# Hunger-Prevails/3D-Pose-Estimation-with-Previleged-Information

Hardware: AMD Instinct MI355X
Metric: crops/sec (fwd+bwd) ResNet-50 pose head, 256x256 bs=64/GPU (higher is better)
Workload: dtype f32 (3xbf16 split, 6 products, f32 accumulate); 1 GPU; depthnet resnet50 pose head, 256x256 crops, batch 64/GPU, full step: fwd + soft-argmax + SmoothL1 + bwd + RCCL grad all-reduce + clip + Adam; global_batch=64, parallelism=dp1, dist_world_size=1, wgrad_stream_runs_beside_launch_stream=True

## Files before the change

### 3d-pose-estimation-with-previleged-information_amd/csrc/p3d_fx.hip

```cpp
#include <type_traits>
#include <mutex>
#include "p3d_common.h"
#include "p3d_fx.h"

namespace p3d {

using bf8 = __bf16 __attribute__((ext_vector_type(8)));
using f32x16 = float __attribute__((ext_vector_type(16)));
using f32x4 = float __attribute__((ext_vector_type(4)));
using f32x2 = float __attribute__((ext_vector_type(2)));
using u32x2 = unsigned __attribute__((ext_vector_type(2)));
using s4t = short __attribute__((ext_vector_type(4)));
using s8v = short __attribute__((ext_vector_type(8)));
using i32x4 = int __attribute__((ext_vector_type(4)));

constexpr int FX_BM = 128, FX_BN = 128, FX_BK = 16;
constexpr int FX_PIECE = 128 * FX_BK * 2;

using bf16x2 = __bf16 __attribute__((ext_vector_type(2)));
__device__ __forceinline__ unsigned fx_pack2(float a, float b) {
    const bf16x2 h = __builtin_convertvector(f32x2{a, b}, bf16x2);
    return __builtin_bit_cast(unsigned, h);
}
__device__ __forceinline__ void fx_split2(float x0, float x1, unsigned& hp, unsigned& mp, unsigned& lp) {
// ... 401 lines not shown
                    if (!split) {
                        const f32x4 c2 = *reinterpret_cast<const f32x4*>(p.ep_c + ((size_t)n * p.M + m) * OHW + rem);
#pragma unroll
                        for (int e = 0; e < 4; ++e) {
                            const float gg = fmaf(c2[e], esc[b], esh[b]) > 0.f ? v[e] : 0.f;
                            ssum[b] += gg; ssq[b] = fmaf(gg, c2[e] - emean[b], ssq[b]);
                        }
                    }
                }
            }
        }
    if (dense) {
        constexpr int EROW = 512 + 16;
        const bool accum = EPI != 3 && !split && p.accumulate;
#pragma unroll
        for (int b = 0; b < 2; ++b) {
            if (b == 1) __syncthreads();
#pragma unroll
            for (int a = 0; a < 2; ++a)
#pragma unroll
                for (int g = 0; g < 4; ++g)
                    *reinterpret_cast<f32x4*>(lds + (wm * 32 + fr) * EROW + (wn * 64 + a * 32 + 8 * g + 4 * fh) * 4) =
                        f32x4{acc[a][b][4 * g], acc[a][b][4 * g + 1], acc[a][b][4 * g + 2], acc[a][b][4 * g + 3]};
            __syncthreads();
#pragma unroll
            for (int i = 0; i < 8; ++i) {
                const int id = t + 256 * i, row = id >> 5, q = id & 31;
                const int m = m0 + (row >> 5) * 64 + b * 32 + (row & 31);
                const int c4 = n0 + 4 * q;
                if (m >= p.M || c4 >= p.NP) continue;
                const int n = c4 / OHW, rem = c4 - n * OHW;
                f32x4 v = *reinterpret_cast<const f32x4*>(lds + row * EROW + q * 16);
                const size_t at = ((size_t)n * p.M + m) * OHW + rem;
                f32x4* dst = reinterpret_cast<f32x4*>(yout + at);
                if (accum) {
                    f32x4 o4;
                    if (p.acc_src) {
                        o4 = *reinterpret_cast<const f32x4*>(p.acc_src + at);
                        if (p.acc_mask) {
                            const unsigned mk = p.acc_mask[at >> 2];
#pragma unroll
                            for (int e = 0; e < 4; ++e) o4[e] = (mk >> e) & 1u ? o4[e] : 0.f;
                        }
                    } else o4 = *dst;
                    v[0] += o4[0]; v[1] += o4[1]; v[2] += o4[2]; v[3] += o4[3];
                }
                if constexpr (EPIX == 8) {
                    if (p.ep_res) { const f32x4 r4 = *reinterpret_cast<const f32x4*>(p.ep_res + at); v[0] += r4[0]; v[1] += r4[1]; v[2] += r4[2]; v[3] += r4[3]; }
                    if (p.ep_relu) { v[0] = fmaxf(v[0], 0.f); v[1] = fmaxf(v[1], 0.f); v[2] = fmaxf(v[2], 0.f); v[3] = fmaxf(v[3], 0.f); }
                }
                *dst = v;
            }
        }
    }
    if constexpr (EPI == 1 || EPI == 2) {
        if (!split) {
#pragma unroll
            for (int b = 0; b < 2; ++b) {
                ssum[b] += __shfl_xor(ssum[b], 32, 64);
                ssq[b] += __shfl_xor(ssq[b], 32, 64);
                if (fh == 0) { red[wn][0][wm * 64 + b * 32 + fr] = ssum[b]; red[wn][1][wm * 64 + b * 32 + fr] = ssq[b]; }
            }
            __syncthreads();
            if (t < 128 && m0 + t < p.M) {
                float* dst = p.partial + ((size_t)tile_n * p.M + m0 + t) * 2;
                dst[0] = red[0][0][t] + red[1][0][t];
                dst[1] = red[0][1][t] + red[1][1][t];
            }
        }
    }
    if constexpr (EPI == 3) {
        float (*const red3)[3][128] = reinterpret_cast<float (*)[3][128]>(lds + 40960);
#pragma unroll
        for (int b = 0; b < 2; ++b) {
            ssum[b] += __shfl_xor(ssum[b], 32, 64);
            ssq[b] += __shfl_xor(ssq[b], 32, 64);
            sthird[b] += __shfl_xor(sthird[b], 32, 64);
            if (fh == 0) { const int ch = wm * 64 + b * 32 + fr; red3[wn][0][ch] = ssum[b]; red3[wn][1][ch] = ssq[b]; red3[wn][2][ch] = sthird[b]; }
        }
        __syncthreads();
        if (t < 128 && m0 + t < p.M)
            *reinterpret_cast<f32x4*>(p.tail_partial + ((size_t)tile_n * p.M + m0 + t) * 4) =
                f32x4{red3[0][0][t] + red3[1][0][t], red3[0][1][t] + red3[1][1][t], red3[0][2][t] + red3[1][2][t], 0.f};
    }
}

template <int BM, int EPI, bool TAPI = false>
__global__ __launch_bounds__(256, 3) void fx16_conv_kernel(const FxConvParams p_in) {
    const FxConvParams p = fx_class_params(p_in);
    static_assert(BM == 128 || BM == 96 || BM == 64, "channel tile");
    constexpr int GA = 4, GB = BM / 32;
    constexpr int WCH = BM / 2;
    constexpr int PIECE_P = 128 * 32, PIECE_C = BM * 32;
    constexpr int BUFB = 3 * PIECE_P + 3 * PIECE_C, CH0 = 3 * PIECE_P;
    constexpr int LDSB = 2 * BUFB > 43008 ? 2 * BUFB : 43008;
    __shared__ __attribute__((aligned(16))) unsigned char lds[LDSB];
    float (*const red)[2][128] = reinterpret_cast<float (*)[2][128]>(lds + 40960);
    const int t = threadIdx.x, lane = t & 63, wave = __builtin_amdgcn_readfirstlane(t >> 6), wm = wave >> 1, wn = wave & 1;
    int bid;
    {
        const int nwg = gridDim.x, q = nwg >> 3, r = nwg & 7, xcd = blockIdx.x & 7, idx = blockIdx.x >> 3;
        bid = (xcd < r ? xcd * (q + 1) : r * (q + 1) + (xcd - r) * q) + idx;
    }
    const int tiles_n_all = gridDim.x / p.tiles_m;
    const int tile_m = p.order ? bid / tiles_n_all : bid % p.tiles_m, tile_n = p.order ? bid % tiles_n_all : bid / p.tiles_m;
    const int m0 = tile_m * BM, n0 = tile_n * FX_BN;
    const int OHW = p.OH * p.OW;
    const int HWi = p.Hi * p.Wi;
    const int nfirst = n0 / OHW;
    const int csteps = p.Cred / FX_BK;
    const int tiles128 = (p.M + 127) >> 7;
    int nk = p.ntap * csteps, kt0 = 0;
    if (p.kchunk > 0) {
        kt0 = blockIdx.y * p.kchunk;
        nk = min(nk - kt0, p.kchunk);
    }
    int f_tap = kt0 / csteps, f_k = (kt0 - f_tap * csteps) * FX_BK;
    if constexpr (TAPI) { f_k = (kt0 / p.ntap) * FX_BK; f_tap = kt0 - (kt0 / p.ntap) * p.ntap; }

    const i32x4 rW = fx_rsrc(p.Wimg, (size_t)p.R * p.S * tiles128 * csteps * (3 * FX_PIECE));
    int w_voff[3], w_lds[3];
#pragma unroll
    for (int j = 0; j < 3; ++j) {
        const int id = t + 256 * j, pc = id / (2 * BM), i = id - pc * (2 * BM), row = i >> 1, half = i & 1;
        const int grow = m0 + row, tl = grow >> 7;
        const bool ok = pc < 3 && tl < tiles128;
        w_voff[j] = ok ? tl * csteps * (3 * FX_PIECE) + pc * FX_PIECE + fx_rc_off(grow & 127, half) : FX_OOB;
        w_lds[j] = CH0 + (pc < 3 ? pc : 0) * PIECE_C + 16 * i;
    }
    constexpr int WCHUNKS = (3 * 2 * BM + 255) / 256;
    const bool w_last = (3 * 2 * BM) % 256 == 0 || t + 256 * (WCHUNKS - 1) < 3 * 2 * BM;

    const int pp = t >> 1, ph = t & 1;
    const int col = n0 + pp;
    const bool col_ok = col < p.NP;
    int hbase = 0, wbase = 0, img_off = 0;
    {
        const int cc = col_ok ? col : 0;
        const int pn = cc / OHW;
        const int rem = cc - pn * OHW, oh = rem / p.OW, ow = rem - oh * p.OW;
        hbase = oh * p.hmul + p.hoff;
        wbase = ow * p.wmul + p.woff;
        img_off = (pn - nfirst) * csteps * HWi;
    }
    i32x4 rXi[3];
    {
        const size_t left = (size_t)(p.N - nfirst) * p.Cred * HWi * 2;
#pragma unroll
        for (int pc = 0; pc < 3; ++pc) rXi[pc] = fx_rsrc(p.Ximg + pc * p.plane_bytes + (size_t)nfirst * p.Cred * HWi * 2, left);
    }
    int x_voff = FX_OOB, w_tapoff = 0, cur_tap = -1;
    auto set_tap = [&](int tap) {
        cur_tap = tap;
        const int ir = tap / p.nS, is = tap - ir * p.nS;
        const int wtap = (p.r0 + p.rstep * ir) * p.S + p.s0 + p.sstep * is;
        w_tapoff = wtap * tiles128 * csteps * (3 * FX_PIECE);
        const int hi = hbase + ir * p.hstep, wi0 = wbase + is * p.wstep;
        const bool ok = col_ok && (unsigned)hi < (unsigned)p.Hi && (unsigned)wi0 < (unsigned)p.Wi;
        x_voff = ok ? (img_off + hi * p.Wi + wi0) * 32 + 16 * ph : FX_OOB;
    };
    i32x4 rwi[3], rxi[3];
    auto fetch = [&]() {
        if (f_tap != cur_tap) { asm volatile("" ::: "memory"); set_tap(f_tap); }
        {
            const int so = w_tapoff + (f_k >> 4) * (3 * FX_PIECE);
#pragma unroll
// ... 782 lines not shown
    }
    const FxPairSide a{c_a, (unsigned char*)img_a, fa->gamma, fa->dgamma, fa->dbeta, fa->table, pixmul_a}, b{c_b, (unsigned char*)img_b, fb->gamma, fb->dgamma, fb->dbeta, fb->table, nullptr};
    const dim3 grid((unsigned)ceil_div((int64_t)N * (HW >> 2) * 2, 256), (unsigned)(C >> 4));
    hipLaunchKernelGGL(fx_act_image_pair_kernel, grid, dim3(256), 0, st, x, gmask, a, b, (const double*)fa->partial, fa->rows, fa->count, fa->accumulate,
                       (size_t)N * C * HW * 2, N, C, HW);
    return check_launch("fx_act_image_pair");
}

size_t fx_act_image_bytes(int64_t N, int64_t C, int64_t HW) { return (size_t)(3 * N * C * HW * 2); }

int32_t fx_act_image(int mode, const float* x, const float* x2, const float* table, int masked, void* img, int N, int C, int HW, hipStream_t st,
                     const FxFinalize* fin, const float* pixmul) {
    if (!x || !img || N <= 0 || C <= 0 || (C & 15) || HW <= 0 || (HW & 3) || (mode != 0 && !table && !fin) || (mode == 2 && !x2) || mode < 0 || mode > 2) {
        set_error("fx_act_image: bad argument (N=%d C=%d HW=%d mode=%d; C %% 16 == 0 and HW %% 4 == 0 are required)", N, C, HW, mode); return P3D_EINVAL;
    }
    FxFinalize f{};
    if (fin) {
        f = *fin;
        if (!((f.kind == 1 && mode == 1 && f.beta) || ((f.kind == 2 || f.kind == 3) && mode == 2 && f.dgamma && f.dbeta)) || !f.partial || f.rows <= 0 || !f.gamma || !f.table) {
            set_error("fx_act_image: inconsistent fused-finalize request (kind %d, mode %d)", f.kind, mode); return P3D_EINVAL;
        }
    }
    const size_t plane = (size_t)N * C * HW * 2;
    const dim3 grid((unsigned)ceil_div((int64_t)N * (HW >> 2) * 2, 256), (unsigned)(C >> 4));
    if (mode == 0) hipLaunchKernelGGL(fx_act_image_kernel<0>, grid, dim3(256), 0, st, x, x2, table, (unsigned char*)img, plane, N, C, HW, masked, f, pixmul);
    else if (mode == 1) hipLaunchKernelGGL(fx_act_image_kernel<1>, grid, dim3(256), 0, st, x, x2, table, (unsigned char*)img, plane, N, C, HW, masked, f, pixmul);
    else hipLaunchKernelGGL(fx_act_image_kernel<2>, grid, dim3(256), 0, st, x, x2, table, (unsigned char*)img, plane, N, C, HW, masked, f, pixmul);
    return check_launch("fx_act_image");
}

static int g_fx = -1;
bool fx_enabled() {
    if (g_fx < 0) { const char* e = getenv("P3D_X3"); g_fx = (e && atoi(e) == 0) ? 0 : 1; }
    return g_fx == 1;
}
int fx_set_enabled(int on) { const int before = fx_enabled() ? 1 : 0; g_fx = on ? 1 : 0; return before; }

static std::mutex g_fx_count_mu;
static unsigned long long g_fx_count[6];
static double g_fx_flops[6];
void fx_count(int kind, const p3d_conv_desc* d) {
    std::lock_guard<std::mutex> lock(g_fx_count_mu);
    g_fx_count[kind] += 1;
    g_fx_flops[kind] += 2.0 * d->N * d->K * d->Ho * d->Wo * (double)d->C * d->R * d->S;
}
void fx_stats(unsigned long long* counts, double* flops, int reset) {
    std::lock_guard<std::mutex> lock(g_fx_count_mu);
    for (int i = 0; i < 6; ++i) { if (counts) counts[i] = g_fx_count[i]; if (flops) flops[i] = g_fx_flops[i]; }
    if (reset) for (int i = 0; i < 6; ++i) { g_fx_count[i] = 0; g_fx_flops[i] = 0.0; }
}

static bool fx_common(const p3d_conv_desc* d) {
    return fx_enabled() && d->c_offset >= 0 && d->c_offset + d->C <= d->c_total && d->R == d->S && (d->R & 1) && d->stride <= 2 &&
           (int64_t)d->N * d->C * d->H * d->W < (1ll << 31) && (int64_t)d->N * d->K * d->Ho * d->Wo < (1ll << 31) &&
           (int64_t)(d->K + 127) * (d->C + 127) * d->R * d->S * 6 < (1ll << 31);
}
bool fx_fwd_applies(const p3d_conv_desc* d, int min_m) {
    return fx_common(d) && d->C % FX_BK == 0 && d->C >= 32 && d->Wo % 4 == 0 && d->W % 4 == 0 && d->K >= min_m;
}
bool fx_dgrad_applies(const p3d_conv_desc* d, int min_m) {
    if (!(fx_common(d) && d->K % FX_BK == 0 && d->K >= 32 && d->C % 4 == 0 && d->C >= min_m && d->Wo % 4 == 0)) return false;
    if (d->stride == 1) return d->W % 4 == 0;
    return d->H % 2 == 0 && d->W % 8 == 0 && d->pad == d->dil * (d->R - 1) / 2 && (d->R == 1 || d->dil == 1);
}
bool fx_wgrad_applies(const p3d_conv_desc* d, int min_m) {
    if ((int64_t)d->N * d->C * d->H * d->W >= (1ll << 29) || (int64_t)d->N * d->K * d->Ho * d->Wo >= (1ll << 29)) return false;
    return fx_common(d) && d->K >= min_m && d->C >= min_m && (d->Ho * d->Wo) % FX_BK == 0 && d->Wo % 4 == 0 && d->W % 4 == 0 && (d->R == 1 || d->C % 64 == 0);
}

static int g_force_conv_splits = 0, g_force_wgrad_splits = 0, g_wgrad_target = 0;
static int g_tap_inner_min = [] { const char* e = getenv("P3D_TAP_INNER_MIN"); return e ? atoi(e) : 1024; }();
static int g_two_taps = 1;
static int g_conv_order = -1, g_wgrad_order = -1;
static int fx_conv_order(size_t wimg_bytes, int tiles_m, int tiles_n) {
    (void)wimg_bytes; (void)tiles_m; (void)tiles_n;
    return g_conv_order > 0 ? 1 : 0;
}
static int fx_wgrad_order(const p3d_conv_desc* d) {
    static const int env = [] { const char* e = getenv("P3D_WGRAD_ORDER"); return e ? atoi(e) : -1; }();
    const int forced = g_wgrad_order >= 0 ? g_wgrad_order : env;
    if (forced >= 0) return forced > 0 ? 1 : 0;
    return (d->R * d->S > 1 && d->C >= 512) ? 1 : 0;
}
static int g_class_launches = 0;
static int g_fx16 = -1;
static int fx16_mode() {
    if (g_fx16 < 0) { const char* e = getenv("P3D_FX16"); g_fx16 = e ? atoi(e) : 1; if (g_fx16 < 0 || g_fx16 > 2) g_fx16 = 1; }
    return g_fx16;
}
static int fx16_bm(int M, bool img, int pro, int epi) {
    const int mode = fx16_mode();
    if (epi == 5 || epi == 6 || epi == 7) epi = epi == 7 ? 0 : epi - 4;
    if (epi == 8) epi = 0;
    if (!img || pro != 0 || (epi != 0 && epi != 1 && epi != 2) || mode == 0) return 0;
    if (M <= 64) return 64;
    if (ceil_div(M, 96) * 96 < ceil_div(M, 128) * 128) return 96;
    return mode == 2 ? 128 : 0;
}
void fx_tune(int what, int value) {
    if (what == 3) { g_pair_map = value; return; }
    if (what == 5) { g_class_launches = value ? 1 : 0; return; }
    if (what == 9) { g_two_taps = value < 0 ? 1 : value; return; }
    if (what == 10) { g_tap_inner_min = value; return; }
    if (what == 7) { g_conv_order = value; return; }
    if (what == 8) { g_wgrad_order = value; return; }
    if (what == 4) { g_fx16 = value < 0 || value > 2 ? 1 : value; return; }
    (what == 0 ? g_force_wgrad_splits : what == 1 ? g_force_conv_splits : g_wgrad_target) = value;
}

struct FxSplit { int splits, kchunk; };
static FxSplit fx_plan_split(int64_t tiles, int nk) {
    FxSplit s{1, 0};
    int64_t want;
    if (g_force_conv_splits > 0) want = g_force_conv_splits < nk ? g_force_conv_splits : nk;
    else {
        static const int target = [] { const char* e = getenv("P3D_SPLITK_BLOCKS"); const int v = e ? atoi(e) : -1; return v >= 0 ? v : 768; }();
        if (tiles > 400 || nk < 64 || target == 0) return s;
        want = ceil_div(target, tiles);
        if (want > nk / 32) want = nk / 32;
        if (want > 8) want = 8;
    }
    if (want < 2) return s;
    s.kchunk = (int)ceil_div(nk, want);
    s.splits = (int)ceil_div(nk, s.kchunk);
    if (s.splits < 2) { s.splits = 1; s.kchunk = 0; }
    return s;
}

size_t fx_weight_image_bytes(int K, int C, int RS, bool bwd) {
    const int rows = bwd ? C : K, red = bwd ? K : C;
    return (size_t)RS * ((rows + 127) / 128) * (red / FX_BK) * (3 * FX_PIECE);
}
static size_t align256(size_t v) { return (v + 255) & ~(size_t)255; }

static FxSplit fx_fwd_split(const p3d_conv_desc* d) {
    return fx_plan_split(ceil_div(d->K, FX_BM) * ceil_div((int64_t)d->N * d->Ho * d->Wo, FX_BN), d->R * d->S * (d->C / FX_BK));
}
static FxSplit fx_dgrad_split(const p3d_conv_desc* d) {
    if (d->stride != 1) return FxSplit{1, 0};
    return fx_plan_split(ceil_div(d->C, FX_BM) * ceil_div((int64_t)d->N * d->H * d->W, FX_BN), d->R * d->S * (d->K / FX_BK));
}
static bool fx_masked_on() { static const bool on = [] { const char* e = getenv("P3D_FX_MASKED"); return !(e && atoi(e) == 0); }(); return on; }
bool fx_fwd_masked_applies(const p3d_conv_desc* d) { return fx_masked_on() && fx_fwd_applies(d, 64); }
bool fx_dgrad_masked_applies(const p3d_conv_desc* d) { return fx_masked_on() && fx_dgrad_applies(d, 64); }
bool fx_wgrad_masked_applies(const p3d_conv_desc* d) { return fx_masked_on() && fx_wgrad_applies(d, 96); }
size_t fx_fwd_workspace(const p3d_conv_desc* d) {
    const FxSplit s = fx_fwd_split(d);
    return align256(fx_weight_image_bytes(d->K, d->C, d->R * d->S, false)) + (s.splits > 1 ? (size_t)s.splits * d->N * d->K * d->Ho * d->Wo * sizeof(float) : 0);
}
size_t fx_dgrad_workspace(const p3d_conv_desc* d) {
    const FxSplit s = fx_dgrad_split(d);
    return align256(fx_weight_image_bytes(d->K, d->C, d->R * d->S, true)) + (s.splits > 1 ? (size_t)s.splits * d->N * d->C * d->H * d->W * sizeof(float) : 0);
}
int fx_partial_rows_fwd(const p3d_conv_desc* d) {
    const FxSplit s = fx_fwd_split(d);
    return s.splits > 1 ? (d->N < 16 ? d->N : 16) : (int)ceil_div((int64_t)d->N * d->Ho * d->Wo, FX_BN);
}
int fx_partial_rows_dgrad(const p3d_conv_desc* d) {
    const FxSplit s = fx_dgrad_split(d);
    return s.splits > 1 ? (d->N < 16 ? d->N : 16) : (int)ceil_div((int64_t)d->N * d->H * d->W, FX_BN);
}

__device__ __forceinline__ void fx_weight_image_chunks(const float* __restrict__ w, unsigned char* __restrict__ img, int K, int C, int RS, bool bwd, size_t first, size_t step,
                                                       int ctot, int coff, const float* __restrict__ scale = nullptr) {
    const int rows = bwd ? C : K, red = bwd ? K : C;
    const int tiles = (rows + 127) / 128, ksteps = red / FX_BK;
    const size_t total = (size_t)RS * tiles * ksteps * 256;
    for (size_t i = first; i < total; i += step) {
        const int half = (int)(i & 1), row = (int)((i >> 1) & 127);
        size_t j = i >> 8;
        const int ks = (int)(j % ksteps); j /= ksteps;
        const int tm = (int)(j % tiles);
        const int tap = (int)(j / tiles);
        const int m = tm * 128 + row, k0 = ks * FX_BK + half * 8;
        unsigned hi[8], mid[8], lo[8];
#pragma unroll
        for (int e = 0; e < 8; ++e) {
            float x = 0.f;
            if (m < rows) x = bwd ? w[((size_t)(k0 + e) * ctot + coff + m) * RS + tap] : w[((size_t)m * ctot + coff + k0 + e) * RS + tap];
            if (scale && m < rows) x = x * scale[m];
            const unsigned hb = __builtin_bit_cast(unsigned, x) & 0xFFFF0000u;
            const float r1 = x - __builtin_bit_cast(float, hb);
            const unsigned mb = __builtin_bit_cast(unsigned, r1) & 0xFFFF0000u;
            const float r2 = r1 - __builtin_bit_cast(float, mb);
            hi[e] = hb; mid[e] = mb; lo[e] = __builtin_bit_cast(unsigned, r2) & 0xFFFF0000u;
        }
        unsigned char* dst = img + (((size_t)tap * tiles + tm) * ksteps + ks) * (3 * FX_PIECE) + fx_rc_off(row, half);
        *reinterpret_cast<i32x4*>(dst) = i32x4{(int)((hi[0] >> 16) | hi[1]), (int)((hi[2] >> 16) | hi[3]), (int)((hi[4] >> 16) | hi[5]), (int)((hi[6] >> 16) | hi[7])};
        *reinterpret_cast<i32x4*>(dst + FX_PIECE) = i32x4{(int)((mid[0] >> 16) | mid[1]), (int)((mid[2] >> 16) | mid[3]), (int)((mid[4] >> 16) | mid[5]), (int)((mid[6] >> 16) | mid[7])};
        *reinterpret_cast<i32x4*>(dst + 2 * FX_PIECE) = i32x4{(int)((lo[0] >> 16) | lo[1]), (int)((lo[2] >> 16) | lo[3]), (int)((lo[4] >> 16) | lo[5]), (int)((lo[6] >> 16) | lo[7])};
    }
}
__global__ __launch_bounds__(256) void fx_weight_images_kernel(const float* __restrict__ w, unsigned char* __restrict__ img_fwd, unsigned char* __restrict__ img_bwd, int K,
                                                               int C, int RS, int ctot, int coff) {
    const bool bwd = blockIdx.y == 1;
    unsigned char* img = bwd ? img_bwd : img_fwd;
    if (img) fx_weight_image_chunks(w, img, K, C, RS, bwd, (size_t)blockIdx.x * 256 + threadIdx.x, (size_t)gridDim.x * 256, ctot, coff);
}
struct FxImageJob { const float* w; unsigned char* fwd; unsigned char* bwd; int K, C, RS, pad; };
__global__ __launch_bounds__(256) void fx_weight_images_batched_kernel(const FxImageJob* __restrict__ jobs) {
    const FxImageJob j = jobs[blockIdx.y >> 1];
    const bool bwd = blockIdx.y & 1;
    unsigned char* img = bwd ? j.bwd : j.fwd;
    if (img) fx_weight_image_chunks(j.w, img, j.K, j.C, j.RS, bwd, (size_t)blockIdx.x * 256 + threadIdx.x, (size_t)gridDim.x * 256, j.C, 0);
}
int32_t fx_build_weight_images_batched(const void* jobs, int njobs, int blocks, hipStream_t st) {
    static_assert(sizeof(FxImageJob) == 40, "job table layout (ops_block.py builds it)");
    if (njobs <= 0) return P3D_OK;
    hipLaunchKernelGGL(fx_weight_images_batched_kernel, dim3((unsigned)(blocks < 1 ? 1 : blocks), (unsigned)(2 * njobs)), dim3(256), 0, st, (const FxImageJob*)jobs);
    return check_launch("fx_build_weight_images_batched");
}

constexpr int FX_FOLD_MAX_K = 2048;
__global__ __launch_bounds__(256) void fx_fold_bn_kernel(const p3d_fold_job* __restrict__ jobs) {
    const p3d_fold_job j = jobs[blockIdx.y];
    __shared__ float sc[FX_FOLD_MAX_K];
    if (j.K <= 0 || j.K > FX_FOLD_MAX_K || j.C <= 0 || j.RS <= 0 || j.c_offset < 0 || j.c_offset + j.C > j.c_total || (j.kind == 0 && j.C % FX_BK != 0)) return;
    const bool bn = j.gamma != nullptr;
    for (int m = threadIdx.x; m < j.K; m += 256) {
        const float s = bn ? j.gamma[m] / sqrtf(j.var[m] + j.eps) : 1.f;
        sc[m] = s;
        if (blockIdx.x == 0 && j.bias_out) {
            float b = bn ? j.beta[m] - j.mean[m] * s : 0.f;
            if (j.conv_bias) b = bn ? b + s * j.conv_bias[m] : j.conv_bias[m];
            j.bias_out[m] = b;
        }
    }
    __syncthreads();
    const size_t first = (size_t)blockIdx.x * 256 + threadIdx.x, step = (size_t)gridDim.x * 256;
    if (j.kind == 0) {
        fx_weight_image_chunks(j.w, (unsigned char*)j.out, j.K, j.C, j.RS, false, first, step, j.c_total, j.c_offset, bn ? sc : nullptr);
    } else {
        float* out = (float*)j.out;
        const size_t per = (size_t)j.C * j.RS, total = (size_t)j.K * per;
        for (size_t i = first; i < total; i += step) {
            const int m = (int)(i / per);
            const size_t rest = i - (size_t)m * per;
            const int c = (int)(rest / j.RS), tap = (int)(rest - (size_t)c * j.RS);
            const float x = j.w[((size_t)m * j.c_total + j.c_offset + c) * j.RS + tap];
            out[i] = bn ? x * sc[m] : x;
        }
    }
}
int32_t fx_fold_bn_images(const void* jobs, int njobs, int blocks, hipStream_t st) {
    static_assert(sizeof(p3d_fold_job) == 96, "job table layout (infer.py builds it)");
    if (njobs <= 0) return P3D_OK;
    hipLaunchKernelGGL(fx_fold_bn_kernel, dim3((unsigned)(blocks < 1 ? 1 : blocks), (unsigned)njobs), dim3(256), 0, st, (const p3d_fold_job*)jobs);
    return check_launch("fx_fold_bn_images");
}

int32_t fx_build_weight_images(const float* w, int K, int C, int RS, void* img_fwd, void* img_bwd, hipStream_t st, int ctot, int coff) {
    if (ctot <= 0) { ctot = C; coff = 0; }
    const size_t a = img_fwd ? fx_weight_image_bytes(K, C, RS, false) / 48 : 0, b = img_bwd ? fx_weight_image_bytes(K, C, RS, true) / 48 : 0;
    const size_t total = a > b ? a : b;
    if (total == 0) return P3D_OK;
    const unsigned blocks = (unsigned)(ceil_div((int64_t)total, 256) < 4096 ? ceil_div((int64_t)total, 256) : 4096);
    hipLaunchKernelGGL(fx_weight_images_kernel, dim3(blocks, 2), dim3(256), 0, st, w, (unsigned char*)img_fwd, (unsigned char*)img_bwd, K, C, RS, ctot, coff);
    return check_launch("fx_build_weight_images");
}

static void fx_launch_conv(const FxConvParams& p_in, bool img, int pro, int epi, int bm, dim3 grid, hipStream_t st) {
    const int am = img ? 1 : 0;
    FxConvParams p = p_in;
    if (p.tap_inner && !((bm == 0 && am == 1 && pro == 0 && epi >= 0 && epi <= 2) || (bm == 96 && epi >= 0 && epi <= 2))) p.tap_inner = 0;
    if (p.tap_inner) {
#define P3D_FX_TAPI(EPI) if (bm == 0 && epi == EPI) { hipLaunchKernelGGL((fx_conv_kernel<1, 0, EPI, true>), grid, dim3(256), 0, st, p); return; } \
                         if (bm == 96 && epi == EPI) { hipLaunchKernelGGL((fx16_conv_kernel<96, EPI, true>), grid, dim3(256), 0, st, p); return; }
        P3D_FX_TAPI(0) P3D_FX_TAPI(1) P3D_FX_TAPI(2)
#undef P3D_FX_TAPI
    }
#define P3D_FX16_CASE(BM, EPI) if (bm == BM && (epi == EPI || epi == (EPI == 0 ? 7 : EPI + 4))) { hipLaunchKernelGGL((fx16_conv_kernel<BM, EPI>), grid, dim3(256), 0, st, p); return; }
    P3D_FX16_CASE(128, 0) P3D_FX16_CASE(128, 1) P3D_FX16_CASE(128, 2)
    P3D_FX16_CASE(96, 0) P3D_FX16_CASE(96, 1) P3D_FX16_CASE(96, 2)
    P3D_FX16_CASE(64, 0) P3D_FX16_CASE(64, 1) P3D_FX16_CASE(64, 2)
    P3D_FX16_CASE(128, 8) P3D_FX16_CASE(96, 8) P3D_FX16_CASE(64, 8)
#undef P3D_FX16_CASE
#define P3D_FX_CASE(AM, PRO, EPI) if (am == AM && pro == PRO && epi == EPI) { hipLaunchKernelGGL((fx_conv_kernel<AM, PRO, EPI>), grid, dim3(256), 0, st, p); return; }
    P3D_FX_CASE(0, 0, 0) P3D_FX_CASE(0, 0, 1) P3D_FX_CASE(0, 0, 2) P3D_FX_CASE(0, 4, 0) P3D_FX_CASE(0, 4, 4) P3D_FX_CASE(0, 4, 5)
    P3D_FX_CASE(1, 0, 0) P3D_FX_CASE(1, 0, 1) P3D_FX_CASE(1, 0, 2) P3D_FX_CASE(1, 0, 3) P3D_FX_CASE(1, 0, 5) P3D_FX_CASE(1, 0, 6) P3D_FX_CASE(1, 0, 7)
    P3D_FX_CASE(0, 0, 8) P3D_FX_CASE(1, 0, 8)
#undef P3D_FX_CASE
    set_error("fx_launch_conv: no kernel instance for img=%d pro=%d epi=%d bm=%d", am, pro, epi, bm);
}

static void fx_launch_reduce(int epi, dim3 grid, hipStream_t st, const float* slabs, float* y, const float* bias, int nsplit, size_t slab_stride, int N, int M,
                             int OHW, int accumulate, const float* ep_c, const float* ep_tab, float* partial, const float* emask, const float* res = nullptr,
                             int relu = 0) {
    if (epi == 5 || epi == 6 || epi == 7 || epi == 4 || epi == 8) epi = epi == 5 ? 1 : epi == 6 ? 2 : 0;
    prof_kernel_done(st);
    if (epi == 1) hipLaunchKernelGGL(fx_reduce_kernel<1>, grid, dim3(256), 0, st, slabs, y, bias, nsplit, slab_stride, N, M, OHW, accumulate, ep_c, ep_tab, partial, emask, res, relu);
    else if (epi == 2) hipLaunchKernelGGL(fx_reduce_kernel<2>, grid, dim3(256), 0, st, slabs, y, bias, nsplit, slab_stride, N, M, OHW, accumulate, ep_c, ep_tab, partial, emask, res, relu);
    else hipLaunchKernelGGL(fx_reduce_kernel<0>, grid, dim3(256), 0, st, slabs, y, bias, nsplit, slab_stride, N, M, OHW, accumulate, ep_c, ep_tab, partial, emask, res, relu);
}

int32_t fx_conv_fwd(const p3d_conv_desc* d, const float* x, const float* w, const float* bias, float* y, void* workspace, size_t workspace_bytes,
                    const FxFuse* fuse, hipStream_t st) {
    const bool img = fuse && fuse->act_img;
    const bool masked = fuse && (fuse->pmask || fuse->emask);
    const bool infer = fuse && fuse->infer;
    const void* wimg = fuse ? fuse->wimg : nullptr;
    if (masked && (!fuse->emask || bias || (img ? fuse->pmask != nullptr : fuse->pmask == nullptr))) {
        set_error("fx_conv_fwd: the partial-convolution instances take the output factor, the input factor exactly for an fp32 operand, and no bias"); return P3D_EINVAL;
    }
    P3D_REQUIRE(!wimg || (d->c_offset == 0 && d->c_total == d->C), "fx_conv_fwd: a cached weight image with a channel window (c_offset %d, c_total %d, C %d)",
                d->c_offset, d->c_total, d->C);
    P3D_REQUIRE(!infer || (!masked && !fuse->partial && wimg), "fx_conv_fwd: the inference epilogue takes a cached folded weight image and no other fusion");
    P3D_REQUIRE(!(fuse && (fuse->res || fuse->relu)) || infer, "fx_conv_fwd: a residual / ReLU needs the inference epilogue");
    const size_t need = fx_fwd_workspace(d);
    if (need && (!workspace || workspace_bytes < need)) { set_error("fx_conv_fwd: workspace %zu B < required %zu B", workspace_bytes, need); return P3D_EWORKSPACE; }
    FxConvParams p{};
    p.X = x; p.Y = y; p.bias = bias;
    if (img) { p.Ximg = (const unsigned char*)fuse->act_img; p.plane_bytes = (size_t)d->N * d->C * d->H * d->W * 2; }
    p.N = d->N; p.Cred = d->C; p.Hi = d->H; p.Wi = d->W; p.M = d->K; p.OH = d->Ho; p.OW = d->Wo; p.NP = d->N * d->Ho * d->Wo;
    p.YH = d->Ho; p.YW = d->Wo; p.oy0 = 0; p.ox0 = 0; p.oys = 1; p.oxs = 1;
    p.R = d->R; p.S = d->S; p.nR = d->R; p.nS = d->S; p.ntap = d->R * d->S; p.r0 = 0; p.rstep = 1; p.s0 = 0; p.sstep = 1;
    p.hmul = d->stride; p.hoff = -d->pad; p.hstep = d->dil; p.wmul = d->stride; p.woff = -d->pad; p.wstep = d->dil;
    p.accumulate = d->accumulate;
    const int RS = d->R * d->S;
    char* ws = (char*)workspace;
    if (!wimg) {
        if (int32_t e = fx_build_weight_images(w, d->K, d->C, RS, ws, nullptr, st, d->c_total, d->c_offset)) return e;
        wimg = ws;
    }
    ws += align256(fx_weight_image_bytes(d->K, d->C, RS, false));
    p.Wimg = (const unsigned char*)wimg;
    int pro = 0, epi = 0;
    if (fuse) {
        if (fuse->partial) { epi = 1; p.partial = fuse->partial; }
        if (masked) { pro = img ? 0 : 4; epi = fuse->partial ? 5 : (img ? 7 : 4); p.pmask = fuse->pmask; p.emask = fuse->emask; }
        if (infer) { epi = 8; p.ep_res = fuse->res; p.ep_relu = fuse->relu; }
    }
    const int tiles_n = (int)ceil_div(p.NP, FX_BN);
    const FxSplit sp = fx_fwd_split(d);
    const int bm = fx16_bm(d->K, img, sp.splits > 1 ? 0 : pro, sp.splits > 1 ? 0 : epi);
    p.tiles_m = (int)ceil_div(d->K, bm ? bm : FX_BM);
    p.order = fx_conv_order(fx_weight_image_bytes(d->K, d->C, RS, false), p.tiles_m, tiles_n);
    p.tap_inner = img && RS > 1 && g_tap_inner_min > 0 && d->C >= g_tap_inner_min;
    if (sp.splits > 1) {
        p.kchunk = sp.kchunk; p.slab_stride = (size_t)d->N * d->K * d->Ho * d->Wo; p.Y = (float*)ws; p.bias = nullptr;
        const float* em = p.emask;
        p.emask = nullptr;
        fx_launch_conv(p, img, pro == 4 ? 4 : 0, 0, bm, dim3((unsigned)(p.tiles_m * tiles_n), (unsigned)sp.splits), st);
        fx_launch_reduce(epi, dim3((unsigned)d->K, (unsigned)(d->N < 16 ? d->N : 16)), st, (const float*)ws, y, bias, sp.splits, p.slab_stride, d->N, d->K,
                         d->Ho * d->Wo, d->accumulate, nullptr, nullptr, p.partial, em, p.ep_res, p.ep_relu);
    } else {
        fx_launch_conv(p, img, pro, epi, bm, dim3((unsigned)(p.tiles_m * tiles_n), 1), st);
    }
    return check_launch("fx_conv_fwd");
}

int32_t fx_conv_dgrad(const p3d_conv_desc* d, const float* dy, const float* w, float* dx, void* workspace, size_t workspace_bytes, const FxFuse* fuse,
                      hipStream_t st) {
    const bool img = fuse && fuse->act_img;
    const bool masked = fuse && (fuse->pmask || fuse->emask);
    const void* wimg = fuse ? fuse->wimg : nullptr;
    P3D_REQUIRE(!wimg || (d->c_offset == 0 && d->c_total == d->C), "fx_conv_dgrad: a cached weight image with a channel window (c_offset %d, c_total %d, C %d)",
                d->c_offset, d->c_total, d->C);
    if (masked && (!fuse->emask || (img ? fuse->pmask != nullptr : fuse->pmask == nullptr) || (!img && fuse->partial))) {
        set_error("fx_conv_dgrad: the partial-convolution instances take the result factor and the operand factor exactly for an fp32 operand"); return P3D_EINVAL;
    }
    const size_t need = fx_dgrad_workspace(d);
    if (need && (!workspace || workspace_bytes < need)) { set_error("fx_conv_dgrad: workspace %zu B < required %zu B", workspace_bytes, need); return P3D_EWORKSPACE; }
    if (fuse && fuse->acc_src && !(d->accumulate && fx_dgrad_accumulates_from_source(d))) {
        set_error("fx_conv_dgrad: an accumulation source needs accumulate = 1, stride 1 and an unsplit launch"); return P3D_EINVAL;
    }
    FxConvParams p{};
    p.X = dy; p.Y = dx;
    if (img) { p.Ximg = (const unsigned char*)fuse->act_img; p.plane_bytes = (size_t)d->N * d->K * d->Ho * d->Wo * 2; }
    p.N = d->N; p.Cred = d->K; p.Hi = d->Ho; p.Wi = d->Wo; p.M = d->C;
    p.YH = d->H; p.YW = d->W;
    p.R = d->R; p.S = d->S;
    p.accumulate = d->accumulate;
    const int RS = d->R * d->S;
    char* ws = (char*)workspace;
    if (!wimg) {
        if (int32_t e = fx_build_weight_images(w, d->K, d->C, RS, nullptr, ws, st, d->c_total, d->c_offset)) return e;
        wimg = ws;
    }
    ws += align256(fx_weight_image_bytes(d->K, d->C, RS, true));
    p.Wimg = (const unsigned char*)wimg;
    int pro = 0, epi = 0;
    if (fuse) {
        if (fuse->partial) { epi = 2; p.partial = fuse->partial; p.ep_c = fuse->ep_c; p.ep_tab = fuse->ep_tab; }
        if (masked) { pro = img ? 0 : 4; epi = fuse->partial ? 6 : (img ? 7 : 4); p.pmask = fuse->pmask; p.emask = fuse->emask; }
    }
    const bool dsplit = d->stride == 1 && fx_dgrad_split(d).splits > 1;
    static const int tap_inner_bwd = [] { const char* e = getenv("P3D_TAP_INNER_MIN_BWD"); return e ? atoi(e) : -1; }();
    const int ti_min = tap_inner_bwd >= 0 ? tap_inner_bwd : g_tap_inner_min;
    p.tap_inner = img && RS > 1 && ti_min > 0 && d->K >= ti_min;
    if (fuse && fuse->tail_c) {
        if (!(img && epi == 0 && pro == 0 && fx_dgrad_tail_applies(d) && fuse->tail_tab && fuse->tail_partial && (!fuse->tail_rc || fuse->tail_rtab))) {
            set_error("fx_conv_dgrad: the tail sums need an image-fed, dense, unsplit stride-1 data gradient without a BatchNorm epilogue (fx_dgrad_tail_applies)"); return P3D_EINVAL;
        }
        epi = 3;
        p.tail_c = fuse->tail_c; p.tail_tab = fuse->tail_tab; p.tail_rc = fuse->tail_rc; p.tail_rtab = fuse->tail_rtab; p.tail_mask = fuse->tail_mask; p.tail_partial = fuse->tail_partial;
    }
    const int bm = fx16_bm(d->C, img, dsplit ? 0 : pro, dsplit ? 0 : epi);
    p.tiles_m = (int)ceil_div(d->C, bm ? bm : FX_BM);
    if (d->stride == 1) {
        p.OH = d->H; p.OW = d->W; p.NP = d->N * d->H * d->W; p.oy0 = 0; p.ox0 = 0; p.oys = 1; p.oxs = 1;
        p.nR = d->R; p.nS = d->S; p.ntap = RS; p.r0 = 0; p.rstep = 1; p.s0 = 0; p.sstep = 1;
        p.hmul = 1; p.hoff = d->pad; p.hstep = -d->dil; p.wmul = 1; p.woff = d->pad; p.wstep = -d->dil;
        const int tiles_n = (int)ceil_div(p.NP, FX_BN);
        const FxSplit sp = fx_dgrad_split(d);
        p.order = fx_conv_order(fx_weight_image_bytes(d->K, d->C, RS, true), p.tiles_m, tiles_n);
        if (sp.splits > 1) {
            p.kchunk = sp.kchunk; p.slab_stride = (size_t)d->N * d->C * d->H * d->W; p.Y = (float*)ws;
            const float* em = p.emask;
            p.emask = nullptr;
            fx_launch_conv(p, img, pro == 4 ? 4 : 0, 0, bm, dim3((unsigned)(p.tiles_m * tiles_n), (unsigned)sp.splits), st);
            fx_launch_reduce(epi, dim3((unsigned)d->C, (unsigned)(d->N < 16 ? d->N : 16)), st, (const float*)ws, dx, nullptr, sp.splits, p.slab_stride, d->N, d->C,
                             d->H * d->W, d->accumulate, p.ep_c, p.ep_tab, p.partial, em);
        } else {
            if (fuse && fuse->acc_src && d->accumulate) { p.acc_src = fuse->acc_src; p.acc_mask = fuse->acc_mask; }
            fx_launch_conv(p, img, pro, epi, bm, dim3((unsigned)(p.tiles_m * tiles_n), 1), st);
        }
        return check_launch("fx_conv_dgrad");
    }
    if (epi != 0 && epi != 4 && epi != 7) { set_error("fx_conv_dgrad: the BatchNorm-backward epilogue is not available for strided data gradients"); return P3D_EINVAL; }
    const int st2 = d->stride;
    p.OH = d->H / st2; p.OW = d->W / st2; p.NP = d->N * p.OH * p.OW; p.oys = st2; p.oxs = st2;
    p.hmul = 1; p.wmul = 1;
    const int tiles_n = (int)ceil_div(p.NP, FX_BN);
    FxConvClass cls[4];
    int ncls = 0;
    for (int ph = 0; ph < st2; ++ph)
        for (int pw = 0; pw < st2; ++pw) {
            int nr = 0, ns = 0, r0 = -1, r1 = -1, q0 = -1, q1 = -1;
            for (int r = 0; r < d->R; ++r) { const int tt = ph + d->pad - r * d->dil; if (((tt % st2) + st2) % st2 == 0) { if (r0 < 0) r0 = r; else if (r1 < 0) r1 = r; ++nr; } }
            for (int s = 0; s < d->S; ++s) { const int tt = pw + d->pad - s * d->dil; if (((tt % st2) + st2) % st2 == 0) { if (q0 < 0) q0 = s; else if (q1 < 0) q1 = s; ++ns; } }
            if (nr == 0 || ns == 0) continue;
            FxConvParams c = p;
            c.nR = nr; c.nS = ns; c.ntap = nr * ns; c.r0 = r0; c.rstep = r1 < 0 ? 1 : r1 - r0; c.s0 = q0; c.sstep = q1 < 0 ? 1 : q1 - q0;
            const int th = ph + d->pad - r0 * d->dil, tw = pw + d->pad - q0 * d->dil;
            c.hoff = th >= 0 ? th / st2 : -((-th) / st2); c.hstep = -(c.rstep * d->dil) / st2;
            c.woff = tw >= 0 ? tw / st2 : -((-tw) / st2); c.wstep = -(c.sstep * d->dil) / st2;
            c.oy0 = ph; c.ox0 = pw;
            if (g_class_launches) { fx_launch_conv(c, img, pro, epi, bm, dim3((unsigned)(c.tiles_m * tiles_n), 1), st); continue; }
            cls[ncls++] = FxConvClass{c.nR, c.nS, c.ntap, c.r0, c.rstep, c.s0, c.sstep, c.hoff, c.hstep, c.woff, c.wstep, c.oy0, c.ox0};
        }
    if (ncls > 0) {
        for (int i = 1; i < ncls; ++i)
            for (int j = i; j > 0 && cls[j].ntap > cls[j - 1].ntap; --j) { const FxConvClass t = cls[j]; cls[j] = cls[j - 1]; cls[j - 1] = t; }
        p.ncls = ncls;
        for (int i = 0; i < ncls; ++i) p.cls[i] = cls[i];
        fx_launch_conv(p, img, pro, epi, bm, dim3((unsigned)(p.tiles_m * tiles_n), 1, (unsigned)ncls), st);
    }
    return check_launch("fx_conv_dgrad");
}

bool fx_dgrad_tail_applies(const p3d_conv_desc* d) {
    return fx_dgrad_applies(d, 96) && d->stride == 1 && fx_dgrad_split(d).splits == 1 && (d->H * d->W) % 4 == 0 && fx16_bm(d->C, true, 0, 0) == 0;
}
int fx_dgrad_tail_rows(const p3d_conv_desc* d) { return (int)ceil_div((int64_t)d->N * d->H * d->W, FX_BN); }
__global__ __launch_bounds__(64) void fx_tail_fold_kernel(const float* __restrict__ partial, int rows, int C, double* __restrict__ sums, int out_rows) {
    const int c = blockIdx.x * 64 + threadIdx.x, r = blockIdx.y;
    if (c >= C) return;
    double s0 = 0.0, s1 = 0.0, s2 = 0.0;
    for (int i = r; i < rows; i += out_rows) {
        const f32x4 v = *reinterpret_cast<const f32x4*>(partial + ((size_t)i * C + c) * 4);
        s0 += v[0]; s1 += v[1]; s2 += v[2];
    }
    double* dst = sums + ((size_t)c * out_rows + r) * 3;
    dst[0] = s0; dst[1] = s1; dst[2] = s2;
}
int32_t fx_tail_fold(const float* partial, int rows, int C, double* sums, int out_rows, hipStream_t st) {
    hipLaunchKernelGGL(fx_tail_fold_kernel, dim3((unsigned)ceil_div(C, 64), (unsigned)out_rows), dim3(64), 0, st, partial, rows, C, sums, out_rows);
    return check_launch("fx_tail_fold");
}

bool fx_dgrad_has_dead_classes(const p3d_conv_desc* d) { return d->stride > 1 && d->R == 1; }
bool fx_dgrad_accumulates_from_source(const p3d_conv_desc* d) { return d->stride == 1 && fx_dgrad_split(d).splits == 1 && (d->H * d->W) % 4 == 0; }

int fx_wgrad_two_taps(const p3d_conv_desc* d, bool images) {
    static const int env = [] { const char* e = getenv("P3D_TWO_TAPS"); return e ? atoi(e) : 1; }();
    if (!g_two_taps || !env || !images || d->C != 64 || d->R * d->S <= 1 || (d->Wo & 15)) return 0;
    return (g_two_taps == 1 && env == 1 && d->K <= 64) ? 3 : 2;
}
int fx_wgrad_splits(const p3d_conv_desc* d, bool images) {
    const int tt = fx_wgrad_two_taps(d, images);
    const int64_t tiles = tt ? ceil_div(d->K, FX_BM) * ceil_div(d->R * d->S, tt) : ceil_div(d->K, FX_BM) * ceil_div(d->C, FX_BN) * d->R * d->S;
    const int64_t total = (int64_t)d->N * (d->Ho * d->Wo / FX_BK);
    int64_t target;
    if (g_wgrad_target > 0) target = g_wgrad_target;
    else if (tiles >= 256) target = 1536;
    else switch ((int)tiles) {
        case 2: target = 384; break;
        case 4: target = 640; break;
        case 5: target = 512; break;
        case 8: case 32: case 36: target = 512; break;
        case 16: target = 256; break;
        case 128: target = 1024; break;
        case 144: target = 720; break;
        default: target = 768;
    }
    static const int scale = [] { const char* e = getenv("P3D_WGRAD_SCALE"); const int v = e ? atoi(e) : 0; return v > 0 ? v : 100; }();
    target = target * scale / 100;
    int64_t splits = (2 * target + tiles) / (2 * tiles);
// ... 188 lines not shown
```

Baseline: 2335 crops/s.

## Add persistent streaming kernel for bandwidth-bound 1x1 convolutions

Adds a persistent grid-strided kernel for 1x1 stride-1 forward and data-gradient convolutions. Each block walks its column tiles and all channel tiles in one continuous software pipeline, so the K loop never drains between output tiles. Output is staged through LDS for coalesced stores, with the fused epilogues kept. A roofline heuristic picks this path only for layers it judges memory-bound. The cost is more LDS per block, lower occupancy (launch bounds 2), and a fixed 512-block grid that may leave compute units idle or unevenly loaded.

```diff
diff --git a/3d-pose-estimation-with-previleged-information_amd/csrc/p3d_fx.hip b/3d-pose-estimation-with-previleged-information_amd/csrc/p3d_fx.hip
--- a/3d-pose-estimation-with-previleged-information_amd/csrc/p3d_fx.hip
+++ b/3d-pose-estimation-with-previleged-information_amd/csrc/p3d_fx.hip
@@ -507,6 +507,249 @@
         if (t < 128 && m0 + t < p.M)
             *reinterpret_cast<f32x4*>(p.tail_partial + ((size_t)tile_n * p.M + m0 + t) * 4) =
                 f32x4{red3[0][0][t] + red3[1][0][t], red3[0][1][t] + red3[1][1][t], red3[0][2][t] + red3[1][2][t], 0.f};
+    }
+}
+
+constexpr int FXS_GRID = 512;
+template <int AMODE, int PRO, int EPIX>
+__global__ __launch_bounds__(256, 2) void fx_stream_kernel(const FxConvParams p) {
+    constexpr int EPI = EPIX == 5 ? 1 : EPIX == 6 ? 2 : EPIX == 7 || EPIX == 4 ? 0 : EPIX;
+    constexpr bool EM = EPIX >= 4 && EPIX <= 7;
+    static_assert(AMODE == 0 || PRO == 0, "the partial-convolution factor is applied by the in-kernel split");
+    constexpr int BUFB = 6 * FX_PIECE, CH0 = 3 * FX_PIECE;
+    constexpr int EROW = 512 + 16, SROWS = 32;
+    __shared__ __attribute__((aligned(16))) unsigned char lds[2 * BUFB + SROWS * EROW];
+    __shared__ float red[2][2][128];
+    unsigned char* const stg = lds + 2 * BUFB;
+    const int t = threadIdx.x, lane = t & 63, wave = __builtin_amdgcn_readfirstlane(t >> 6), wm = wave >> 1, wn = wave & 1;
+    const int HW = p.OH * p.OW;
+    const int csteps = p.Cred / FX_BK;
+    const int tiles_n = (p.NP + FX_BN - 1) / FX_BN;
+    const int G = gridDim.x, blk = blockIdx.x;
+    const int nitems = ((tiles_n - blk + G - 1) / G) * p.tiles_m;
+    const int nk = nitems * csteps;
+
+    const i32x4 rW = fx_rsrc(p.Wimg, (size_t)p.tiles_m * csteps * (3 * FX_PIECE));
+    int w_voff[3];
+#pragma unroll
+    for (int j = 0; j < 3; ++j) w_voff[j] = 16 * (t + 256 * j);
+    const int trow = t >> 5, tp4 = t & 31;
+    const int pp = t >> 1, ph = (t & 1) ^ ((t >> 4) & 1);
+    i32x4 rX, rXi[3];
+    if constexpr (AMODE == 0) rX = fx_rsrc(p.X, (size_t)p.N * p.Cred * HW * sizeof(float));
+    else {
+#pragma unroll
+        for (int pc = 0; pc < 3; ++pc) rXi[pc] = fx_rsrc(p.Ximg + pc * p.plane_bytes, (size_t)p.N * p.Cred * HW * 2);
+    }
+    const i32x4 rPM = fx_rsrc(PRO == 4 ? p.pmask : nullptr, PRO == 4 ? (size_t)p.N * HW * sizeof(float) : 0);
+
+    int f_item = 0, f_k = 0, x_voff = FX_OOB, w_item = 0;
+    f32x4 tmask = {1.f, 1.f, 1.f, 1.f}, smask = {1.f, 1.f, 1.f, 1.f};
+    auto set_item = [&](int item) {
+        const int j = item / p.tiles_m, tm = item - j * p.tiles_m;
+        w_item = tm * csteps * (3 * FX_PIECE);
+        const int col = (blk + G * j) * FX_BN + (AMODE == 0 ? 4 * tp4 : pp);
+        x_voff = FX_OOB;
+        if (col < p.NP) {
+            const int pn = col / HW, rem = col - pn * HW;
+            x_voff = AMODE == 0 ? ((pn * p.Cred + trow) * HW + rem) * 4 : (pn * csteps * HW + rem) * 32 + 16 * ph;
+        }
+        if constexpr (PRO == 4) tmask = fx_buffer_load_f32x4(rPM, x_voff >= 0 ? col * 4 : FX_OOB, 0, 0);
+    };
+    f32x4 rx[2];
+    i32x4 rwi[3], rxi[3];
+    auto fetch = [&]() {
+        if (f_k == 0) { asm volatile("" ::: "memory"); set_item(f_item); }
+        {
+            const int so = w_item + (f_k >> 4) * (3 * FX_PIECE);
+#pragma unroll
+            for (int j = 0; j < 3; ++j) rwi[j] = fx_buffer_load_i32x4(rW, w_voff[j], so, 0);
+        }
+        if constexpr (AMODE != 0) {
+            const int so = (f_k >> 4) * HW * 32;
+#pragma unroll
+            for (int pc = 0; pc < 3; ++pc) rxi[pc] = fx_buffer_load_i32x4(rXi[pc], x_voff, so, 0);
+        } else {
+#pragma unroll
+            for (int i = 0; i < 2; ++i) rx[i] = fx_buffer_load_f32x4(rX, x_voff, (f_k + 8 * i) * HW * 4, 0);
+            if constexpr (PRO == 4) smask = tmask;
+        }
+        f_k += FX_BK;
+        if (f_k == p.Cred) { f_k = 0; ++f_item; }
+    };
+    const int st_p[2] = {fx_tr_off(trow, tp4 >> 1) + 8 * (tp4 & 1), fx_tr_off(trow + 8, tp4 >> 1) + 8 * (tp4 & 1)};
+    const int st_p1 = fx_rc_off(pp, ph);
+    auto stage = [&](int buf) {
+        unsigned char* pb = lds + buf * BUFB;
+        unsigned char* cb = pb + CH0;
+#pragma unroll
+        for (int j = 0; j < 3; ++j) *reinterpret_cast<i32x4*>(cb + 16 * (t + 256 * j)) = rwi[j];
+        if constexpr (AMODE != 0) {
+#pragma unroll
+            for (int pc = 0; pc < 3; ++pc) *reinterpret_cast<i32x4*>(pb + pc * FX_PIECE + st_p1) = rxi[pc];
+        } else {
+#pragma unroll
+            for (int i = 0; i < 2; ++i) {
+                f32x4 v = rx[i];
+                if constexpr (PRO == 4) {
+#pragma unroll
+                    for (int e = 0; e < 4; ++e) v[e] *= smask[e];
+                }
+                fx_split_store(pb + st_p[i], v);
+            }
+        }
+    };
+
+    f32x16 acc[2][2];
+    auto zero_acc = [&]() {
+#pragma unroll
+        for (int a = 0; a < 2; ++a)
+#pragma unroll
+            for (int b = 0; b < 2; ++b)
+#pragma unroll
+                for (int r = 0; r < 16; ++r) acc[a][b][r] = 0.f;
+    };
+    zero_acc();
+    const int fr = lane & 31, fh = lane >> 5;
+    int rd_p[2][2], rd_c[2];
+#pragma unroll
+    for (int a = 0; a < 2; ++a) {
+        if constexpr (AMODE == 0) fx_tr_frag_off(lane, wn * 64 + a * 32, rd_p[a]);
+        else rd_p[a][0] = rd_p[a][1] = fx_rc_off(wn * 64 + a * 32 + fr, fh);
+        rd_c[a] = CH0 + fx_rc_off(wm * 64 + a * 32 + fr, fh);
+    }
+
+    auto epilogue = [&](int item) {
+        const int j = item / p.tiles_m, tm = item - j * p.tiles_m;
+        const int n0 = (blk + G * j) * FX_BN, m0 = tm * FX_BM;
+        float ssum[2] = {0.f, 0.f}, ssq[2] = {0.f, 0.f};
+        float esc[2] = {0.f, 0.f}, esh[2] = {0.f, 0.f}, emean[2] = {0.f, 0.f};
+        if constexpr (EPI == 2) {
+#pragma unroll
+            for (int b = 0; b < 2; ++b) {
+                const int m = m0 + wm * 64 + b * 32 + fr;
+                esc[b] = p.ep_tab[8 * m]; esh[b] = p.ep_tab[8 * m + 1]; emean[b] = p.ep_tab[8 * m + 2];
+            }
+        }
+#pragma unroll
+        for (int a = 0; a < 2; ++a)
+#pragma unroll
+            for (int g = 0; g < 4; ++g) {
+                const int c4 = n0 + wn * 64 + a * 32 + 8 * g + 4 * fh;
+                if (c4 >= p.NP) continue;
+                const int n = c4 / HW, rem = c4 - n * HW;
+#pragma unroll
+                for (int b = 0; b < 2; ++b) {
+                    const int m = m0 + wm * 64 + b * 32 + fr;
+                    f32x4 v = {acc[a][b][4 * g], acc[a][b][4 * g + 1], acc[a][b][4 * g + 2], acc[a][b][4 * g + 3]};
+                    if constexpr (EM) {
+                        const f32x4 em = *reinterpret_cast<const f32x4*>(p.emask + (size_t)n * HW + rem);
+                        v[0] *= em[0]; v[1] *= em[1]; v[2] *= em[2]; v[3] *= em[3];
+                    }
+#pragma unroll
+                    for (int e = 0; e < 4; ++e) acc[a][b][4 * g + e] = v[e];
+                    if constexpr (EPI == 1) {
+#pragma unroll
+                        for (int e = 0; e < 4; ++e) { ssum[b] += v[e]; ssq[b] = fmaf(v[e], v[e], ssq[b]); }
+                    }
+                    if constexpr (EPI == 2) {
+                        const f32x4 c2 = *reinterpret_cast<const f32x4*>(p.ep_c + ((size_t)n * p.M + m) * HW + rem);
+#pragma unroll
+                        for (int e = 0; e < 4; ++e) {
+                            const float gg = fmaf(c2[e], esc[b], esh[b]) > 0.f ? v[e] : 0.f;
+                            ssum[b] += gg; ssq[b] = fmaf(gg, c2[e] - emean[b], ssq[b]);
+                        }
+                    }
+                }
+            }
+#pragma unroll
+        for (int b = 0; b < 2; ++b)
+#pragma unroll
+            for (int h = 0; h < 2; ++h) {
+                if (wm == h) {
+#pragma unroll
+                    for (int a = 0; a < 2; ++a)
+#pragma unroll
+                        for (int g = 0; g < 4; ++g)
+                            *reinterpret_cast<f32x4*>(stg + fr * EROW + (wn * 64 + a * 32 + 8 * g + 4 * fh) * 4) =
+                                f32x4{acc[a][b][4 * g], acc[a][b][4 * g + 1], acc[a][b][4 * g + 2], acc[a][b][4 * g + 3]};
+                }
+                __syncthreads();
+                auto store_round = [&](auto accb) {
+#pragma unroll
+                for (int i = 0; i < 4; ++i) {
+                    const int id = t + 256 * i, row = id >> 5, q = id & 31;
+                    const int m = m0 + h * 64 + b * 32 + row;
+                    const int c4 = n0 + 4 * q;
+                    if (c4 >= p.NP) continue;
+                    const int n = c4 / HW, rem = c4 - n * HW;
+                    f32x4 v = *reinterpret_cast<const f32x4*>(stg + row * EROW + q * 16);
+                    const size_t at = ((size_t)n * p.M + m) * HW + rem;
+                    f32x4* dst = reinterpret_cast<f32x4*>(p.Y + at);
+                    if constexpr (decltype(accb)::value) {
+                        f32x4 o4;
+                        if (p.acc_src) {
+                            o4 = *reinterpret_cast<const f32x4*>(p.acc_src + at);
+                            if (p.acc_mask) {
+                                const unsigned mk = p.acc_mask[at >> 2];
+#pragma unroll
+                                for (int e = 0; e < 4; ++e) o4[e] = (mk >> e) & 1u ? o4[e] : 0.f;
+                            }
+                        } else o4 = *dst;
+                        v[0] += o4[0]; v[1] += o4[1]; v[2] += o4[2]; v[3] += o4[3];
+                    }
+                    *dst = v;
+                }
+                };
+                if (p.accumulate) store_round(std::true_type{});
+                else store_round(std::false_type{});
+                __syncthreads();
+            }
+        if constexpr (EPI == 1 || EPI == 2) {
+#pragma unroll
+            for (int b = 0; b < 2; ++b) {
+                ssum[b] += __shfl_xor(ssum[b], 32, 64);
+                ssq[b] += __shfl_xor(ssq[b], 32, 64);
+                if (fh == 0) { red[wn][0][wm * 64 + b * 32 + fr] = ssum[b]; red[wn][1][wm * 64 + b * 32 + fr] = ssq[b]; }
+            }
+            __syncthreads();
+            if (t < 128) {
+                float* dst = p.partial + ((size_t)(blk + G * j) * p.M + m0 + t) * 2;
+                dst[0] = red[0][0][t] + red[1][0][t];
+                dst[1] = red[0][1][t] + red[1][1][t];
+            }
+        }
+        zero_acc();
+    };
+
+    if (nk > 0) { fetch(); stage(0); if (nk > 1) fetch(); }
+    __syncthreads();
+    bf8 pf[3][2], cf[3][2];
+    for (int kt = 0; kt < nk; ++kt) {
+        const int buf = kt & 1;
+        const unsigned char* bb = lds + buf * BUFB;
+        auto read_p = [&](int pc) {
+#pragma unroll
+            for (int a = 0; a < 2; ++a) {
+                if constexpr (AMODE == 0) pf[pc][a] = fx_tr_read(bb + pc * FX_PIECE, rd_p[a]);
+                else pf[pc][a] = *reinterpret_cast<const bf8*>(bb + pc * FX_PIECE + rd_p[a][0]);
+            }
+        };
+        auto read_c = [&](int pc) {
+#pragma unroll
+            for (int a = 0; a < 2; ++a) cf[pc][a] = *reinterpret_cast<const bf8*>(bb + pc * FX_PIECE + rd_c[a]);
+        };
+        read_p(2); read_c(0); read_p(0); read_c(2);
+        __builtin_amdgcn_sched_barrier(0);
+        P3D_FX_PRODUCTS_RANGE(acc, pf, cf, 2, 2, 0, 1)
+        __builtin_amdgcn_sched_barrier(0);
+        if (kt + 1 < nk) stage(buf ^ 1);
+        if (kt + 2 < nk) fetch();
+        __builtin_amdgcn_sched_barrier(0);
+        read_p(1); read_c(1);
+        P3D_FX_PRODUCTS_RANGE(acc, pf, cf, 2, 2, 1, 6)
+        __syncthreads();
+        if (kt - (kt / csteps) * csteps == csteps - 1) epilogue(kt / csteps);
     }
 }
 
@@ -1455,6 +1698,7 @@
     if (forced >= 0) return forced > 0 ? 1 : 0;
     return (d->R * d->S > 1 && d->C >= 512) ? 1 : 0;
 }
+static int g_stream = [] { const char* e = getenv("P3D_FX_STREAM"); return e ? (atoi(e) != 0 ? 1 : 0) : 1; }();
 static int g_class_launches = 0;
 static int g_fx16 = -1;
 static int fx16_mode() {
@@ -1477,6 +1721,7 @@
     if (what == 10) { g_tap_inner_min = value; return; }
     if (what == 7) { g_conv_order = value; return; }
     if (what == 8) { g_wgrad_order = value; return; }
+    if (what == 11) { g_stream = value ? 1 : 0; return; }
     if (what == 4) { g_fx16 = value < 0 || value > 2 ? 1 : value; return; }
     (what == 0 ? g_force_wgrad_splits : what == 1 ? g_force_conv_splits : g_wgrad_target) = value;
 }
@@ -1524,6 +1769,17 @@
 size_t fx_dgrad_workspace(const p3d_conv_desc* d) {
     const FxSplit s = fx_dgrad_split(d);
     return align256(fx_weight_image_bytes(d->K, d->C, d->R * d->S, true)) + (s.splits > 1 ? (size_t)s.splits * d->N * d->C * d->H * d->W * sizeof(float) : 0);
+}
+static bool fx_stream_applies(const p3d_conv_desc* d, bool dgrad) {
+    if (!g_stream || d->R != 1 || d->S != 1 || d->stride != 1 || d->pad != 0) return false;
+    const int64_t red = dgrad ? d->K : d->C, rows = dgrad ? d->C : d->K, HW = (int64_t)d->H * d->W;
+    if (rows % FX_BM != 0 || red % FX_BK != 0 || HW % 4 != 0 || d->N * red * HW * 4 >= (1ll << 31)) return false;
+    if ((dgrad ? fx_dgrad_split(d) : fx_fwd_split(d)).splits > 1) return false;
+    return (double)(red + rows) * 4.0 / 6e12 >= 0.8 * 2.0 * (double)red * rows / 215e12;
+}
+static int fx_stream_grid(const p3d_conv_desc* d) {
+    const int64_t tiles_n = ceil_div((int64_t)d->N * d->H * d->W, FX_BN);
+    return (int)(tiles_n < FXS_GRID ? tiles_n : FXS_GRID);
 }
 int fx_partial_rows_fwd(const p3d_conv_desc* d) {
     const FxSplit s = fx_fwd_split(d);
@@ -1654,6 +1910,15 @@
     P3D_FX_CASE(0, 0, 8) P3D_FX_CASE(1, 0, 8)
 #undef P3D_FX_CASE
     set_error("fx_launch_conv: no kernel instance for img=%d pro=%d epi=%d bm=%d", am, pro, epi, bm);
+}
+
+static void fx_launch_stream(const FxConvParams& p, bool img, int pro, int epi, int blocks, hipStream_t st) {
+    const int am = img ? 1 : 0;
+#define P3D_FXS_CASE(AM, PRO, EPI) if (am == AM && pro == PRO && epi == EPI) { hipLaunchKernelGGL((fx_stream_kernel<AM, PRO, EPI>), dim3((unsigned)blocks), dim3(256), 0, st, p); return; }
+    P3D_FXS_CASE(0, 0, 0) P3D_FXS_CASE(0, 0, 1) P3D_FXS_CASE(0, 0, 2) P3D_FXS_CASE(0, 4, 4) P3D_FXS_CASE(0, 4, 5)
+    P3D_FXS_CASE(1, 0, 0) P3D_FXS_CASE(1, 0, 1) P3D_FXS_CASE(1, 0, 2) P3D_FXS_CASE(1, 0, 5) P3D_FXS_CASE(1, 0, 6) P3D_FXS_CASE(1, 0, 7)
+#undef P3D_FXS_CASE
+    set_error("fx_launch_stream: no kernel instance for img=%d pro=%d epi=%d", am, pro, epi);
 }
 
 static void fx_launch_reduce(int epi, dim3 grid, hipStream_t st, const float* slabs, float* y, const float* bias, int nsplit, size_t slab_stride, int N, int M,
@@ -1716,6 +1981,9 @@
         fx_launch_conv(p, img, pro == 4 ? 4 : 0, 0, bm, dim3((unsigned)(p.tiles_m * tiles_n), (unsigned)sp.splits), st);
         fx_launch_reduce(epi, dim3((unsigned)d->K, (unsigned)(d->N < 16 ? d->N : 16)), st, (const float*)ws, y, bias, sp.splits, p.slab_stride, d->N, d->K,
                          d->Ho * d->Wo, d->accumulate, nullptr, nullptr, p.partial, em, p.ep_res, p.ep_relu);
+    } else if (epi != 8 && !bias && fx_stream_applies(d, false)) {
+        p.tiles_m = d->K / FX_BM;
+        fx_launch_stream(p, img, pro, epi, fx_stream_grid(d), st);
     } else {
         fx_launch_conv(p, img, pro, epi, bm, dim3((unsigned)(p.tiles_m * tiles_n), 1), st);
     }
@@ -1786,7 +2054,10 @@
                              d->H * d->W, d->accumulate, p.ep_c, p.ep_tab, p.partial, em);
         } else {
             if (fuse && fuse->acc_src && d->accumulate) { p.acc_src = fuse->acc_src; p.acc_mask = fuse->acc_mask; }
-            fx_launch_conv(p, img, pro, epi, bm, dim3((unsigned)(p.tiles_m * tiles_n), 1), st);
+            if (epi != 3 && fx_stream_applies(d, true)) {
+                p.tiles_m = d->C / FX_BM;
+                fx_launch_stream(p, img, pro, epi, fx_stream_grid(d), st);
+            } else fx_launch_conv(p, img, pro, epi, bm, dim3((unsigned)(p.tiles_m * tiles_n), 1), st);
         }
         return check_launch("fx_conv_dgrad");
     }
```

Result: no change. 2342 crops/s (median of 6 runs) (+0.3%).
